# parthjaggi/flow

Hardware: AMD Instinct MI355X
Metric: env-steps/sec (higher is better)
Workload: dtype mixed

## Files before the change

flow_amd/csrc/flowsim_pair.h:

```cpp
#pragma once
#include "flowsim_kernels.h"

namespace fs {

typedef float f2 __attribute__((ext_vector_type(2)));
typedef unsigned u2v __attribute__((__vector_size__(8)));

enum : int { DPP_ROW_NEWBCAST0 = 0x150, DPP_ROW_NEWBCAST8 = 0x158 };

__device__ __forceinline__ f2 fma2(f2 a, f2 b, f2 c) { return __builtin_elementwise_fma(a, b, c); }
__device__ __forceinline__ f2 splat(float a) { return f2{a, a}; }

__device__ __forceinline__ f2 pk_mul(f2 a, f2 b) { return a * b; }
__device__ __forceinline__ f2 pk_add(f2 a, f2 b) { return a + b; }
__device__ __forceinline__ f2 pk_sub(f2 a, f2 b) { return a - b; }
__device__ __forceinline__ f2 pk_fma(f2 a, f2 b, f2 c) { return fma2(a, b, c); }
__device__ __forceinline__ f2 pk_fnma(f2 a, f2 b, f2 c) { return fma2(-a, b, c); }
__device__ __forceinline__ float nonneg_else(float x, float y) {
  const unsigned a = __builtin_bit_cast(unsigned, x), b = __builtin_bit_cast(unsigned, y);
  return __builtin_bit_cast(float, min(a, b));
}

template <int ROW>
__device__ __forceinline__ float next_a(float v, bool last, int lane) {
// ... 112 lines not shown
#define FS_PAIR_A_NZ_PARAM
#include "flowsim_pair_step_a_sm.inc"
#undef FS_PAIR_A_NAME
#undef FS_PAIR_A_NZ
#undef FS_PAIR_A_NZ_PARAM
#define FS_PAIR_A_NAME pair_step_asm_a_sm_nz
#define FS_PAIR_A_NZ 1
#define FS_PAIR_A_NZ_PARAM , f2 nz
#include "flowsim_pair_step_a_sm.inc"
#undef FS_PAIR_A_NAME
#undef FS_PAIR_A_NZ
#undef FS_PAIR_A_NZ_PARAM
__device__ __forceinline__ void pair_step_asm_b(f2& V, f2& X, f2& H, f2& DVL, f2& OV, unsigned& crash_bits, float& sq,
                                                const PairConsts& c) {
  asm volatile(
      "v_sub_f32_e32 v118, v112, v113\n"
      "v_sub_f32_e32 v132, v115, v114\n"
      "v_subrev_f32_dpp v119, v112, v113 row_shl:1 row_mask:0xf bank_mask:0xf bound_ctrl:1\n"
      "v_subrev_f32_dpp v134, v112, v113 row_newbcast:0 row_mask:0xf bank_mask:0xf\n"
      "v_sub_f32_dpp v133, v114, v115 row_shl:1 row_mask:0xf bank_mask:0xf bound_ctrl:1\n"
      "v_sub_f32_dpp v135, v114, v115 row_newbcast:0 row_mask:0xf bank_mask:0xf\n"
      "v_cndmask_b32_e64 v119, v119, v134, %[last]\n"
      "v_cndmask_b32_e64 v133, v133, v135, %[last]\n"
      "v_pk_add_f32 v[126:127], v[132:133], %[L2]\n"
      "v_min_u32_e32 v132, v132, v126\n"
      "v_min_u32_e32 v133, v133, v127\n"
      "v_pk_add_f32 v[116:117], v[132:133], %[lenlead] neg_lo:[0,1] neg_hi:[0,1]\n"
      "v_pk_add_f32 v[126:127], v[116:117], %[gap2] neg_lo:[0,1] neg_hi:[0,1]\n"
      "v_min_f32_e32 v126, v126, v127\n"
      "v_alignbit_b32 %[cb], %[cb], v126, 31\n"
      "v_pk_fma_f32 v[124:125], v[112:113], %[vmask], %[tvm]\n"
      "v_pk_mul_f32 v[124:125], v[124:125], v[124:125]\n"
      "v_add_f32_e32 %[sq], v124, v125\n"
      "v_cvt_f64_f32_e32 v[130:131], v112\n"
      "v_cvt_f64_f32_e32 v[132:133], v113\n"
      "v_mul_f64 v[134:135], v[130:131], %[rcms]\n"
      "v_mul_f64 v[136:137], v[132:133], %[rcms]\n"
      "v_fma_f64 v[130:131], -v[134:135], %[ms], v[130:131]\n"
      "v_fma_f64 v[132:133], -v[136:137], %[ms], v[132:133]\n"
      "v_fma_f64 v[134:135], v[130:131], %[rcms], v[134:135]\n"
      "v_fma_f64 v[136:137], v[132:133], %[rcms], v[136:137]\n"
      "v_cvt_f32_f64_e32 v128, v[134:135]\n"
      "v_cvt_f32_f64_e32 v129, v[136:137]\n"
      : "+{v[112:113]}"(V), "+{v[114:115]}"(X), "+{v[116:117]}"(H), "+{v[118:119]}"(DVL), "={v[128:129]}"(OV),
        [cb] "+v"(crash_bits), [sq] "=&v"(sq)
      : [L2] "v"(c.L2), [lenlead] "v"(c.len_lead), [gap2] "v"(c.gap2), [vmask] "v"(c.vmask), [tvm] "v"(c.tvm),
        [ms] "v"(c.ms64), [rcms] "v"(c.rc_ms64), [last] "s"(c.last_mask)
      : "v124", "v125", "v126", "v127", "v130", "v131", "v132", "v133", "v134", "v135", "v136", "v137");
}

struct MixedConsts {
  f2 p0, p1, p2, p5, rc_v0, tsab, rc_ab, one, gap2, vmask, tvm;
  float c1e3;
  double dt, ramp, L, rc_L, rc_ms, len_b, len_next, zero;
  unsigned long long last_mask;
};
__device__ __forceinline__ void mixed_step_asm_a(f2& V32, double& XA, double& XB, double& VA, double& VB, f2& H, f2& DVL,
                                                 f2& OV, const MixedConsts& c) {
  unsigned long long sa, sb;
  asm volatile(
      "v_cmp_nlt_f32_e64 %[sa], |v140|, %[c1e3]\n"
      "v_cmp_nlt_f32_e64 %[sb], |v141|, %[c1e3]\n"
      "v_pk_mul_f32 v[124:125], v[112:113], v[142:143]\n"
      "v_pk_mul_f32 v[126:127], v[124:125], %[rcab]\n"
      "v_pk_fma_f32 v[130:131], v[126:127], %[tsab], v[124:125] neg_lo:[1,0,0] neg_hi:[1,0,0]\n"
      "v_pk_fma_f32 v[126:127], v[130:131], %[rcab], v[126:127]\n"
      "v_cndmask_b32_e64 v120, %[c1e3], v140, %[sa]\n"
      "v_cndmask_b32_e64 v121, %[c1e3], v141, %[sb]\n"
      "v_pk_mul_f32 v[124:125], v[112:113], %[rcv0]\n"
      "v_rcp_f32_e32 v122, v120\n"
      "v_rcp_f32_e32 v123, v121\n"
      "v_pk_fma_f32 v[130:131], v[124:125], %[p0], v[112:113] neg_lo:[1,0,0] neg_hi:[1,0,0]\n"
      "v_pk_fma_f32 v[124:125], v[130:131], %[rcv0], v[124:125]\n"
      "v_pk_mul_f32 v[130:131], v[112:113], %[p1]\n"
      "v_pk_add_f32 v[130:131], v[130:131], v[126:127]\n"
      "v_pk_fma_f32 v[126:127], v[120:121], v[122:123], %[one] neg_lo:[1,0,0] neg_hi:[1,0,0]\n"
      "v_max_f32_e32 v130, 0, v130\n"
      "v_max_f32_e32 v131, 0, v131\n"
      "v_pk_fma_f32 v[122:123], v[126:127], v[122:123], v[122:123]\n"
      "v_pk_add_f32 v[130:131], %[p5], v[130:131]\n"
      "v_pk_mul_f32 v[124:125], v[124:125], v[124:125]\n"
      "v_pk_mul_f32 v[126:127], v[130:131], v[122:123]\n"
      "v_pk_mul_f32 v[124:125], v[124:125], v[124:125]\n"
      "v_pk_fma_f32 v[132:133], v[120:121], v[126:127], v[130:131] neg_lo:[1,0,0] neg_hi:[1,0,0]\n"
      "v_pk_add_f32 v[124:125], %[one], v[124:125] neg_lo:[0,1] neg_hi:[0,1]\n"
      "v_pk_fma_f32 v[126:127], v[132:133], v[122:123], v[126:127]\n"
      "v_pk_fma_f32 v[132:133], v[120:121], v[126:127], v[130:131] neg_lo:[1,0,0] neg_hi:[1,0,0]\n"
      "v_pk_fma_f32 v[126:127], v[132:133], v[122:123], v[126:127]\n"
      "v_pk_mul_f32 v[126:127], v[126:127], v[126:127]\n"
      "v_pk_add_f32 v[124:125], v[124:125], v[126:127] neg_lo:[0,1] neg_hi:[0,1]\n"
      "v_pk_mul_f32 v[124:125], %[p2], v[124:125]\n"
      "v_cvt_f64_f32_e32 v[130:131], v124\n"
      "v_cvt_f64_f32_e32 v[132:133], v125\n"
      "v_mul_f64 v[130:131], v[130:131], %[dt]\n"
      "v_mul_f64 v[132:133], v[132:133], %[dt]\n"
      "v_add_f64 v[130:131], v[118:119], v[130:131]\n"
      "v_add_f64 v[132:133], v[138:139], v[132:133]\n"
      "v_max_f64 v[130:131], v[130:131], %[zero]\n"
      "v_max_f64 v[132:133], v[132:133], %[zero]\n"
      "v_add_f64 v[130:131], v[130:131], -v[118:119]\n"
      "v_add_f64 v[132:133], v[132:133], -v[138:139]\n"
      "v_mul_f64 v[130:131], v[130:131], %[ramp]\n"
      "v_mul_f64 v[132:133], v[132:133], %[ramp]\n"
      "v_add_f64 v[118:119], v[118:119], v[130:131]\n"
      "v_add_f64 v[138:139], v[138:139], v[132:133]\n"
      "v_mul_f64 v[130:131], v[118:119], %[dt]\n"
      "v_mul_f64 v[132:133], v[138:139], %[dt]\n"
      "v_add_f64 v[130:131], v[114:115], v[130:131]\n"
      "v_add_f64 v[132:133], v[116:117], v[132:133]\n"
      "v_add_f64 v[134:135], v[130:131], -%[L]\n"
      "v_add_f64 v[136:137], v[132:133], -%[L]\n"
      "v_cvt_f32_f64_e32 v112, v[118:119]\n"
      "v_cvt_f32_f64_e32 v113, v[138:139]\n"
      "v_cmp_gt_i32_e64 %[sa], 0, v135\n"
      "v_cmp_gt_i32_e64 %[sb], 0, v137\n"
      "v_mul_f64 v[120:121], v[118:119], %[rcms]\n"
      "v_mul_f64 v[122:123], v[138:139], %[rcms]\n"
      "v_cndmask_b32_e64 v114, v134, v130, %[sa]\n"
      "v_cndmask_b32_e64 v115, v135, v131, %[sa]\n"
      "v_cndmask_b32_e64 v116, v136, v132, %[sb]\n"
      "v_cndmask_b32_e64 v117, v137, v133, %[sb]\n"
      "v_cvt_f32_f64_e32 v128, v[120:121]\n"
      "v_cvt_f32_f64_e32 v129, v[122:123]\n"
      : "+{v[112:113]}"(V32), "+{v[114:115]}"(XA), "+{v[116:117]}"(XB), "+{v[118:119]}"(VA), "+{v[138:139]}"(VB),
        "+{v[140:141]}"(H), "+{v[142:143]}"(DVL), "={v[128:129]}"(OV), [sa] "=&s"(sa), [sb] "=&s"(sb)
      : [c1e3] "v"(c.c1e3), [rcab] "v"(c.rc_ab), [tsab] "v"(c.tsab), [rcv0] "v"(c.rc_v0), [p0] "v"(c.p0),
        [p1] "v"(c.p1), [p2] "v"(c.p2), [p5] "v"(c.p5), [one] "v"(c.one), [dt] "v"(c.dt), [ramp] "v"(c.ramp),
        [L] "v"(c.L), [rcms] "v"(c.rc_ms), [zero] "v"(c.zero)
      : "v120", "v121", "v122", "v123", "v124", "v125", "v126", "v127", "v130", "v131", "v132", "v133", "v134",
        "v135", "v136", "v137");
}
struct MixedSumoConsts { double fl0a, fl0b, adta, adtb, ddta, ddtb; };
__device__ __forceinline__ void mixed_step_asm_a_sm(f2& V32, double& XA, double& XB, double& VA, double& VB, f2& H,
                                                    f2& DVL, f2& OV, const MixedConsts& c, const SumoPair& m,
                                                    const MixedSumoConsts& d) {
  unsigned long long sa, sb;
  asm volatile(
      "v_cmp_nlt_f32_e64 %[sa], |v140|, %[c1e3]\n"
      "v_cmp_nlt_f32_e64 %[sb], |v141|, %[c1e3]\n"
      "v_pk_mul_f32 v[124:125], v[112:113], v[142:143]\n"
      "v_pk_mul_f32 v[126:127], v[124:125], %[rcab]\n"
      "v_pk_mul_f32 v[150:151], v[124:125], %[rcts]\n"
      "v_pk_fma_f32 v[130:131], v[126:127], %[tsab], v[124:125] neg_lo:[1,0,0] neg_hi:[1,0,0]\n"
      "v_pk_fma_f32 v[152:153], v[150:151], %[ts], v[124:125] neg_lo:[1,0,0] neg_hi:[1,0,0]\n"
      "v_pk_fma_f32 v[126:127], v[130:131], %[rcab], v[126:127]\n"
      "v_pk_fma_f32 v[150:151], v[152:153], %[rcts], v[150:151]\n"
      "v_cndmask_b32_e64 v120, %[c1e3], v140, %[sa]\n"
      "v_cndmask_b32_e64 v121, %[c1e3], v141, %[sb]\n"
      "v_max_f32_e32 v146, v140, %[c1e3]\n"
      "v_max_f32_e32 v147, v141, %[c1e3]\n"
      "v_pk_mul_f32 v[124:125], v[112:113], %[rcv0]\n"
      "v_rcp_f32_e32 v122, v120\n"
      "v_rcp_f32_e32 v123, v121\n"
      "v_rcp_f32_e32 v148, v146\n"
      "v_rcp_f32_e32 v149, v147\n"
      "v_pk_fma_f32 v[130:131], v[124:125], %[p0], v[112:113] neg_lo:[1,0,0] neg_hi:[1,0,0]\n"
      "v_pk_mul_f32 v[154:155], v[112:113], %[rcsm]\n"
      "v_pk_fma_f32 v[124:125], v[130:131], %[rcv0], v[124:125]\n"
      "v_pk_fma_f32 v[152:153], v[154:155], %[smax], v[112:113] neg_lo:[1,0,0] neg_hi:[1,0,0]\n"
      "v_pk_mul_f32 v[130:131], v[112:113], %[p1]\n"
      "v_pk_fma_f32 v[154:155], v[152:153], %[rcsm], v[154:155]\n"
      "v_pk_add_f32 v[130:131], v[130:131], v[126:127]\n"
      "v_pk_mul_f32 v[152:153], v[112:113], %[tau]\n"
      "v_pk_fma_f32 v[126:127], v[120:121], v[122:123], %[one] neg_lo:[1,0,0] neg_hi:[1,0,0]\n"
      "v_pk_add_f32 v[150:151], v[152:153], v[150:151]\n"
      "v_pk_fma_f32 v[152:153], v[146:147], v[148:149], %[one] neg_lo:[1,0,0] neg_hi:[1,0,0]\n"
      "v_max_f32_e32 v130, 0, v130\n"
      "v_max_f32_e32 v131, 0, v131\n"
      "v_max_f32_e32 v150, 0, v150\n"
      "v_max_f32_e32 v151, 0, v151\n"
      "v_pk_fma_f32 v[122:123], v[126:127], v[122:123], v[122:123]\n"
      "v_pk_fma_f32 v[148:149], v[152:153], v[148:149], v[148:149]\n"
      "v_pk_add_f32 v[130:131], %[p5], v[130:131]\n"
      "v_pk_add_f32 v[150:151], %[mgap], v[150:151]\n"
      "v_pk_mul_f32 v[124:125], v[124:125], v[124:125]\n"
      "v_pk_mul_f32 v[154:155], v[154:155], v[154:155]\n"
      "v_pk_mul_f32 v[126:127], v[130:131], v[122:123]\n"
      "v_pk_mul_f32 v[152:153], v[150:151], v[148:149]\n"
      "v_pk_mul_f32 v[124:125], v[124:125], v[124:125]\n"
      "v_pk_mul_f32 v[154:155], v[154:155], v[154:155]\n"
      "v_pk_fma_f32 v[132:133], v[120:121], v[126:127], v[130:131] neg_lo:[1,0,0] neg_hi:[1,0,0]\n"
      "v_pk_fma_f32 v[134:135], v[146:147], v[152:153], v[150:151] neg_lo:[1,0,0] neg_hi:[1,0,0]\n"
      "v_pk_add_f32 v[124:125], %[one], v[124:125] neg_lo:[0,1] neg_hi:[0,1]\n"
      "v_pk_add_f32 v[154:155], %[one], v[154:155] neg_lo:[0,1] neg_hi:[0,1]\n"
      "v_pk_fma_f32 v[126:127], v[132:133], v[122:123], v[126:127]\n"
      "v_pk_fma_f32 v[152:153], v[134:135], v[148:149], v[152:153]\n"
      "v_pk_fma_f32 v[132:133], v[120:121], v[126:127], v[130:131] neg_lo:[1,0,0] neg_hi:[1,0,0]\n"
      "v_pk_fma_f32 v[134:135], v[146:147], v[152:153], v[150:151] neg_lo:[1,0,0] neg_hi:[1,0,0]\n"
      "v_pk_fma_f32 v[126:127], v[132:133], v[122:123], v[126:127]\n"
      "v_pk_fma_f32 v[152:153], v[134:135], v[148:149], v[152:153]\n"
      "v_pk_mul_f32 v[126:127], v[126:127], v[126:127]\n"
      "v_pk_mul_f32 v[152:153], v[152:153], v[152:153]\n"
      "v_pk_add_f32 v[124:125], v[124:125], v[126:127] neg_lo:[0,1] neg_hi:[0,1]\n"
      "v_pk_add_f32 v[154:155], v[154:155], v[152:153] neg_lo:[0,1] neg_hi:[0,1]\n"
      "v_pk_mul_f32 v[124:125], %[p2], v[124:125]\n"
      "v_pk_mul_f32 v[154:155], %[maxa], v[154:155]\n"
      "v_cvt_f64_f32_e32 v[130:131], v124\n"
      "v_cvt_f64_f32_e32 v[132:133], v125\n"
      "v_cvt_f64_f32_e32 v[134:135], v154\n"
      "v_cvt_f64_f32_e32 v[136:137], v155\n"
      "v_mul_f64 v[130:131], v[130:131], %[dt]\n"
      "v_mul_f64 v[132:133], v[132:133], %[dt]\n"
      "v_mul_f64 v[134:135], v[134:135], %[dt]\n"
      "v_mul_f64 v[136:137], v[136:137], %[dt]\n"
      "v_add_f64 v[130:131], v[118:119], v[130:131]\n"
      "v_add_f64 v[132:133], v[138:139], v[132:133]\n"
      "v_add_f64 v[134:135], v[118:119], v[134:135]\n"
      "v_add_f64 v[136:137], v[138:139], v[136:137]\n"
      "v_max_f64 v[130:131], v[130:131], %[zero]\n"
      "v_max_f64 v[132:133], v[132:133], %[zero]\n"
      "v_max_f64 v[134:135], v[134:135], %[fl0a]\n"
      "v_max_f64 v[136:137], v[136:137], %[fl0b]\n"
      "v_add_f64 v[130:131], v[130:131], -v[118:119]\n"
      "v_add_f64 v[132:133], v[132:133], -v[138:139]\n"
      "v_mul_f64 v[130:131], v[130:131], %[ramp]\n"
      "v_mul_f64 v[132:133], v[132:133], %[ramp]\n"
      "v_add_f64 v[130:131], v[118:119], v[130:131]\n"
      "v_add_f64 v[132:133], v[138:139], v[132:133]\n"
      "v_min_f64 v[130:131], v[130:131], v[134:135]\n"
      "v_min_f64 v[132:133], v[132:133], v[136:137]\n"
      "v_add_f64 v[134:135], v[118:119], %[adta]\n"
      "v_add_f64 v[136:137], v[138:139], %[adtb]\n"
      "v_min_f64 v[130:131], v[130:131], v[134:135]\n"
      "v_min_f64 v[132:133], v[132:133], v[136:137]\n"
      "v_add_f64 v[134:135], v[118:119], -%[ddta]\n"
      "v_add_f64 v[136:137], v[138:139], -%[ddtb]\n"
      "v_max_f64 v[118:119], v[130:131], v[134:135]\n"
      "v_max_f64 v[138:139], v[132:133], v[136:137]\n"
      "v_mul_f64 v[130:131], v[118:119], %[dt]\n"
      "v_mul_f64 v[132:133], v[138:139], %[dt]\n"
      "v_add_f64 v[130:131], v[114:115], v[130:131]\n"
      "v_add_f64 v[132:133], v[116:117], v[132:133]\n"
      "v_add_f64 v[134:135], v[130:131], -%[L]\n"
      "v_add_f64 v[136:137], v[132:133], -%[L]\n"
      "v_cvt_f32_f64_e32 v112, v[118:119]\n"
      "v_cvt_f32_f64_e32 v113, v[138:139]\n"
      "v_cmp_gt_i32_e64 %[sa], 0, v135\n"
      "v_cmp_gt_i32_e64 %[sb], 0, v137\n"
      "v_mul_f64 v[120:121], v[118:119], %[rcms]\n"
      "v_mul_f64 v[122:123], v[138:139], %[rcms]\n"
      "v_cndmask_b32_e64 v114, v134, v130, %[sa]\n"
      "v_cndmask_b32_e64 v115, v135, v131, %[sa]\n"
      "v_cndmask_b32_e64 v116, v136, v132, %[sb]\n"
      "v_cndmask_b32_e64 v117, v137, v133, %[sb]\n"
      "v_cvt_f32_f64_e32 v128, v[120:121]\n"
      "v_cvt_f32_f64_e32 v129, v[122:123]\n"
      : "+{v[112:113]}"(V32), "+{v[114:115]}"(XA), "+{v[116:117]}"(XB), "+{v[118:119]}"(VA), "+{v[138:139]}"(VB),
        "+{v[140:141]}"(H), "+{v[142:143]}"(DVL), "={v[128:129]}"(OV), [sa] "=&s"(sa), [sb] "=&s"(sb)
      : [c1e3] "v"(c.c1e3), [rcab] "v"(c.rc_ab), [tsab] "v"(c.tsab), [rcv0] "v"(c.rc_v0), [p0] "v"(c.p0),
        [p1] "v"(c.p1), [p2] "v"(c.p2), [p5] "v"(c.p5), [one] "v"(c.one), [dt] "v"(c.dt), [ramp] "v"(c.ramp),
        [L] "v"(c.L), [rcms] "v"(c.rc_ms), [zero] "v"(c.zero), [rcts] "v"(m.rc_ts), [ts] "v"(m.ts),
        [rcsm] "v"(m.rc_smax), [smax] "v"(m.smax), [tau] "v"(m.tau), [mgap] "v"(m.min_gap), [maxa] "v"(m.maxa),
        [fl0a] "v"(d.fl0a), [fl0b] "v"(d.fl0b), [adta] "v"(d.adta), [adtb] "v"(d.adtb), [ddta] "v"(d.ddta),
        [ddtb] "v"(d.ddtb)
      : "v120", "v121", "v122", "v123", "v124", "v125", "v126", "v127", "v130", "v131", "v132", "v133", "v134",
        "v135", "v136", "v137", "v146", "v147", "v148", "v149", "v150", "v151", "v152", "v153", "v154", "v155");
}
__device__ __forceinline__ void mixed_step_asm_b(f2& V32, double& XA, double& XB, f2& H, f2& DVL, f2& OX,
                                                 unsigned& crash_bits, float& sq, const MixedConsts& c) {
  unsigned long long sa, sb;
  asm volatile(
      "v_sub_f32_e32 v142, v112, v113\n"
      "v_subrev_f32_dpp v143, v112, v113 row_shl:1 row_mask:0xf bank_mask:0xf bound_ctrl:1\n"
      "v_subrev_f32_dpp v124, v112, v113 row_newbcast:0 row_mask:0xf bank_mask:0xf\n"
      "v_mov_b32_dpp v130, v114 row_shl:1 row_mask:0xf bank_mask:0xf bound_ctrl:1\n"
      "v_mov_b32_dpp v131, v115 row_shl:1 row_mask:0xf bank_mask:0xf bound_ctrl:1\n"
      "v_mov_b32_dpp v132, v114 row_newbcast:0 row_mask:0xf bank_mask:0xf\n"
      "v_mov_b32_dpp v133, v115 row_newbcast:0 row_mask:0xf bank_mask:0xf\n"
      "v_cndmask_b32_e64 v143, v143, v124, %[last]\n"
      "v_cndmask_b32_e64 v130, v130, v132, %[last]\n"
      "v_cndmask_b32_e64 v131, v131, v133, %[last]\n"
      "v_mul_f64 v[120:121], v[114:115], %[rcL]\n"
      "v_mul_f64 v[122:123], v[116:117], %[rcL]\n"
      "v_add_f64 v[134:135], v[116:117], -v[114:115]\n"
      "v_add_f64 v[136:137], v[130:131], -v[116:117]\n"
      "v_cvt_f32_f64_e32 v144, v[120:121]\n"
      "v_cvt_f32_f64_e32 v145, v[122:123]\n"
      "v_add_f64 v[130:131], v[134:135], %[L]\n"
      "v_add_f64 v[132:133], v[136:137], %[L]\n"
      "v_cmp_gt_i32_e64 %[sa], 0, v135\n"
      "v_cmp_gt_i32_e64 %[sb], 0, v137\n"
      "v_pk_fma_f32 v[124:125], v[112:113], %[vmask], %[tvm]\n"
      "v_pk_mul_f32 v[124:125], v[124:125], v[124:125]\n"
      "v_cndmask_b32_e64 v134, v134, v130, %[sa]\n"
      "v_cndmask_b32_e64 v135, v135, v131, %[sa]\n"
      "v_cndmask_b32_e64 v136, v136, v132, %[sb]\n"
      "v_cndmask_b32_e64 v137, v137, v133, %[sb]\n"
      "v_add_f32_e32 %[sq], v124, v125\n"
      "v_add_f64 v[134:135], v[134:135], -%[lenb]\n"
      "v_add_f64 v[136:137], v[136:137], -%[lennext]\n"
      "v_cvt_f32_f64_e32 v140, v[134:135]\n"
      "v_cvt_f32_f64_e32 v141, v[136:137]\n"
      "v_pk_add_f32 v[126:127], v[140:141], %[gap2] neg_lo:[0,1] neg_hi:[0,1]\n"
      "v_min_f32_e32 v126, v126, v127\n"
      "v_alignbit_b32 %[cb], %[cb], v126, 31\n"
      : "+{v[112:113]}"(V32), "+{v[114:115]}"(XA), "+{v[116:117]}"(XB), "+{v[140:141]}"(H), "+{v[142:143]}"(DVL),
        "={v[144:145]}"(OX), [cb] "+v"(crash_bits), [sq] "=&v"(sq), [sa] "=&s"(sa), [sb] "=&s"(sb)
      : [L] "v"(c.L), [rcL] "v"(c.rc_L), [gap2] "v"(c.gap2), [vmask] "v"(c.vmask), [tvm] "v"(c.tvm),
        [lenb] "v"(c.len_b), [lennext] "v"(c.len_next), [last] "s"(c.last_mask)
      : "v120", "v121", "v122", "v123", "v124", "v125", "v126", "v127", "v130", "v131", "v132", "v133", "v134",
        "v135", "v136", "v137");
}

template <typename T, int ROW, bool DELTA4, bool FASTDIV, bool BADCHK, bool SM = false, bool NOISE = false>
__global__ __launch_bounds__(256) void k_rollout_pair(DevView<T> s, int num_steps, float* __restrict__ obs,
                                                      float* __restrict__ rew, uint8_t* __restrict__ done) {
  constexpr bool MIXED = sizeof(T) == 8;
  static_assert(!(NOISE && MIXED), "FS_MIXED has no noise form (its C twin cannot reproduce the hardware's log / cos)");
  constexpr bool ASM = ROW == 16 && DELTA4 && FASTDIV && !BADCHK;
  constexpr int RPW = 64 / ROW;
  constexpr int PERIOD = ROW < 16 ? ROW : 16;
  const int lane = threadIdx.x & 63;
  const int wave = (blockIdx.x * blockDim.x + threadIdx.x) >> 6;
  const int row = lane / ROW;
  const int k = lane % ROW;
  const int r = wave * RPW + row;
  const int N = s.N;
  const int LP = N >> 1;
  const bool rvalid = r < s.R;
  const bool valid = rvalid && k < LP;
  const int rr = rvalid ? r : s.R - 1;
  const int kk = k < LP ? k : LP - 1;
  const bool last = (kk == LP - 1);
  const int iA = 2 * kk, iB = iA + 1;
  const size_t idx = size_t(rr) * N + iA;

  f2 p[6];
#pragma unroll
  for (int q = 0; q < 6; ++q) p[q] = f2{float(s.p[q * N + iA]), float(s.p[q * N + iB])};
  const T lenB = s.length[iB];
  const T len_nextA = next_a<ROW>(T(s.length[iA]), last, lane);
  const T base_len = s.ring_len[rr];
  const T L = base_len + T(4) * s.jlen;
  int tcount = s.time[rr];
  uint32_t nctr = NOISE ? s.noise_ctr[rr] : 0u;
  const f2 sigma = NOISE ? f2{float(s.noise[iA]), float(s.noise[iB])} : f2{0.0f, 0.0f};
  const bool noisyA = NOISE && sigma.x > 0.0f, noisyB = NOISE && sigma.y > 0.0f;
  float gA[4] = {0.0f, 0.0f, 0.0f, 0.0f}, gB[4] = {0.0f, 0.0f, 0.0f, 0.0f};
  if constexpr (NOISE) {
    if ((nctr & 3u) != 0u) {
      gauss4<float>(s.seed_lo, s.seed_hi, s.rep0 + uint32_t(rr), uint32_t(iA), nctr >> 2, gA, s.noise_exact != 0);
      gauss4<float>(s.seed_lo, s.seed_hi, s.rep0 + uint32_t(rr), uint32_t(iB), nctr >> 2, gB, s.noise_exact != 0);
      for (uint32_t q = 0; q < (nctr & 3u); ++q) {
        gA[0] = gA[1]; gA[1] = gA[2]; gA[2] = gA[3];
        gB[0] = gB[1]; gB[1] = gB[2]; gB[2] = gB[3];
      }
    }
  }

  const float dt = float(s.dt), ramp = float(s.ramp);
  const f2 two_sqrt_ab = {2.0f * tsqrt(p[2].x * p[3].x), 2.0f * tsqrt(p[2].y * p[3].y)};
  const f2 rc_v0 = {1.0f / p[0].x, 1.0f / p[0].y}, rc_ab = {1.0f / two_sqrt_ab.x, 1.0f / two_sqrt_ab.y};
  const float Lf = float(L);
  const f2 L2 = splat(Lf), rc_L2 = splat(1.0f / Lf), one = splat(1.0f), dt2 = splat(dt), ramp2 = splat(ramp);
  const f2 gap2 = splat(float(s.crash_gap)), m100 = splat(-100.0f);
  const f2 vmask = splat(valid ? 1.0f : 0.0f), tvm = splat(valid ? -float(s.target_velocity) : 0.0f);
  const double ms64 = double(s.max_speed), rc_ms64 = 1.0 / ms64;
  const double L64 = double(L), rc_L64 = 1.0 / L64, dt64 = double(s.dt), ramp64 = double(s.ramp);

  f2 x, v;
  double xdA = 0, xdB = 0, vdA = 0, vdB = 0;
  if (MIXED) {
    xdA = double(s.pos[idx]); xdB = double(s.pos[idx + 1]);
    vdA = double(s.vel[idx]); vdB = double(s.vel[idx + 1]);
    v = f2{float(vdA), float(vdB)};
    x = f2{0.0f, 0.0f};
  } else {
    x = f2{float(s.pos[idx]), float(s.pos[idx + 1])};
    v = f2{float(s.vel[idx]), float(s.vel[idx + 1])};
  }
  const f2 len_lead = {float(lenB), float(len_nextA)};

  auto headway = [&]() -> f2 {
    if (MIXED) {
      const double xn = next_a<ROW>(xdA, last, lane);
      double dA = xdB - xdA, dB = xn - xdB;
      dA = dA < 0.0 ? dA + L64 : dA;
      dB = dB < 0.0 ? dB + L64 : dB;
      return f2{float(dA - double(lenB)), float(dB - double(len_nextA))};
    } else {
      const f2 xl = {x.y, next_a<ROW>(x.x, last, lane)};
      f2 d = pk_sub(xl, x);
      const f2 dw = pk_add(d, L2);
      d.x = nonneg_else(d.x, dw.x);
      d.y = nonneg_else(d.y, dw.y);
      return pk_sub(d, len_lead);
    }
  };
  f2 h = headway();
  f2 vl = {v.y, next_a<ROW>(v.x, last, lane)};
  f2 dvl = v - vl;
  PairConsts pc;
  pc.p0 = p[0]; pc.p1 = p[1]; pc.p2 = p[2]; pc.p5 = p[5]; pc.rc_v0 = rc_v0; pc.tsab = two_sqrt_ab; pc.rc_ab = rc_ab;
  pc.one = one; pc.dt2 = dt2; pc.ramp2 = ramp2; pc.L2 = L2; pc.rc_L2 = rc_L2; pc.len_lead = len_lead;
  pc.gap2 = gap2; pc.vmask = vmask; pc.tvm = tvm; pc.c1e3 = 1e-3f; pc.ms64 = ms64; pc.rc_ms64 = rc_ms64;
  pc.last_mask = __ballot(last);
  MixedConsts mc;
  mc.p0 = p[0]; mc.p1 = p[1]; mc.p2 = p[2]; mc.p5 = p[5]; mc.rc_v0 = rc_v0; mc.tsab = two_sqrt_ab; mc.rc_ab = rc_ab;
  mc.one = one; mc.gap2 = gap2; mc.vmask = vmask; mc.tvm = tvm; mc.c1e3 = 1e-3f; mc.dt = dt64; mc.ramp = ramp64;
  mc.L = L64; mc.rc_L = rc_L64; mc.rc_ms = rc_ms64; mc.len_b = double(lenB); mc.len_next = double(len_nextA);
  mc.zero = 0.0; mc.last_mask = pc.last_mask;
  SumoPair sc{};
  double floor0A = 0, floor0B = 0, adtA = 0, adtB = 0, ddtA = 0, ddtB = 0;
  if constexpr (SM) {
    const int mA = s.speed_mode[iA], mB = s.speed_mode[iB];
    const float maA = float(s.max_accel[iA]), maB = float(s.max_accel[iB]);
    const float mdA = float(s.max_decel[iA]), mdB = float(s.max_decel[iB]);
    sc.tau = f2{float(s.sumo_tau[iA]), float(s.sumo_tau[iB])};
    sc.min_gap = f2{float(s.sumo_min_gap[iA]), float(s.sumo_min_gap[iB])};
    sc.maxa = f2{maA, maB};
    sc.smax = f2{float(s.sumo_max_speed[iA]), float(s.sumo_max_speed[iB])};
    sc.rc_smax = f2{1.0f / sc.smax.x, 1.0f / sc.smax.y};
    sc.ts = f2{2.0f * tsqrt(maA * mdA), 2.0f * tsqrt(maB * mdB)};
    sc.rc_ts = f2{1.0f / sc.ts.x, 1.0f / sc.ts.y};
    const float BIG = 3.0e38f;
    sc.floor0 = f2{(mA & 1) ? 0.0f : BIG, (mB & 1) ? 0.0f : BIG};
    sc.adt = f2{(mA & 2) ? maA * dt : BIG, (mB & 2) ? maB * dt : BIG};
    sc.ddt = f2{(mA & 4) ? mdA * dt : BIG, (mB & 4) ? mdB * dt : BIG};
    floor0A = double(sc.floor0.x); floor0B = double(sc.floor0.y);
    adtA = (mA & 2) ? double(s.max_accel[iA]) * dt64 : double(BIG);
    adtB = (mB & 2) ? double(s.max_accel[iB]) * dt64 : double(BIG);
    ddtA = (mA & 4) ? double(s.max_decel[iA]) * dt64 : double(BIG);
    ddtB = (mB & 4) ? double(s.max_decel[iB]) * dt64 : double(BIG);
  }
  const MixedSumoConsts msc = {floor0A, floor0B, adtA, adtB, ddtA, ddtB};

  const unsigned rowb = 2u * unsigned(N) * 4u;
  const unsigned off_v = unsigned(rr) * rowb + unsigned(iA) * 4u;
  const unsigned off_x = off_v + unsigned(N) * 4u;
  const size_t step_bytes = size_t(s.R) * rowb;
  const unsigned step_b32 = unsigned(step_bytes);
  char* ob = reinterpret_cast<char*>(obs);
  unsigned crash_bits = 0u, bad_bits = 0u;

  typedef unsigned u4v __attribute__((__vector_size__(16)));
  constexpr bool XPOSE = ASM;
  __shared__ float row_img[XPOSE ? 4 : 1][XPOSE ? RPW * 64 : 1];
  float* const my_img = row_img[XPOSE ? (threadIdx.x >> 6) & 3 : 0] + (XPOSE ? row * 2 * N : 0);
  const unsigned off_16 = unsigned(rr) * rowb + unsigned(kk) * 16u;
  u4v piece = {0u, 0u, 0u, 0u};
  auto transpose_in = [&](f2 ov, f2 ox) {
    *reinterpret_cast<f2*>(my_img + 2 * kk) = ov;
    *reinterpret_cast<f2*>(my_img + N + 2 * kk) = ox;
    __builtin_amdgcn_fence(__ATOMIC_RELEASE, "wavefront");
    __builtin_amdgcn_wave_barrier();
    __builtin_amdgcn_fence(__ATOMIC_ACQUIRE, "wavefront");
    piece = *reinterpret_cast<const u4v*>(my_img + 4 * kk);
  };

  auto noise_term = [&]() -> f2 {
    f2 nz = {-0.0f, -0.0f};
    if constexpr (NOISE) {
      const bool fresh = (nctr & 3u) == 0u;
      if (__ballot(fresh) != 0ull) {
        if (fresh) {
          gauss4<float>(s.seed_lo, s.seed_hi, s.rep0 + uint32_t(rr), uint32_t(iA), nctr >> 2, gA, s.noise_exact != 0);
          gauss4<float>(s.seed_lo, s.seed_hi, s.rep0 + uint32_t(rr), uint32_t(iB), nctr >> 2, gB, s.noise_exact != 0);
        }
      }
      const float tA = sigma.x * gA[0], tB = sigma.y * gB[0];
      nz.x = noisyA ? tA : -0.0f;
      nz.y = noisyB ? tB : -0.0f;
      gA[0] = gA[1]; gA[1] = gA[2]; gA[2] = gA[3];
      gB[0] = gB[1]; gB[1] = gB[2]; gB[2] = gB[3];
      nctr += 1u;
    }
    return nz;
  };

  auto one_step = [&](int slot, __amdgpu_buffer_rsrc_t rs, float& sq_out) {
    if constexpr (ASM) {
      f2 ov, ox;
      const unsigned so = unsigned(slot) * step_b32;
      if constexpr (MIXED) {
        if constexpr (SM) mixed_step_asm_a_sm(v, xdA, xdB, vdA, vdB, h, dvl, ov, mc, sc, msc);
        else mixed_step_asm_a(v, xdA, xdB, vdA, vdB, h, dvl, ov, mc);
        if (slot > 0) __builtin_amdgcn_raw_buffer_store_b128(piece, rs, off_16, so - step_b32, 0);
        mixed_step_asm_b(v, xdA, xdB, h, dvl, ox, crash_bits, sq_out, mc);
        transpose_in(ov, ox);
      } else {
#if defined(FS_DIAG_NOSTORE)
        pair_step_asm_a(v, x, h, dvl, ox, pc);
        pair_step_asm_b(v, x, h, dvl, ov, crash_bits, sq_out, pc);
        asm volatile("" :: "v"(ov), "v"(ox), "s"(so));
#elif defined(FS_DIAG_NOXPOSE)
        pair_step_asm_a(v, x, h, dvl, ox, pc);
        __builtin_amdgcn_raw_buffer_store_b64(__builtin_bit_cast(u2v, ox), rs, off_x, so, 0);
        pair_step_asm_b(v, x, h, dvl, ov, crash_bits, sq_out, pc);
        __builtin_amdgcn_raw_buffer_store_b64(__builtin_bit_cast(u2v, ov), rs, off_v, so, 0);
#else
        if constexpr (NOISE) {
          const f2 nz = noise_term();
          if constexpr (SM) pair_step_asm_a_sm_nz(v, x, h, dvl, ox, pc, sc, nz);
          else pair_step_asm_a_nz(v, x, h, dvl, ox, pc, nz);
        } else {
          if constexpr (SM) pair_step_asm_a_sm(v, x, h, dvl, ox, pc, sc);
          else pair_step_asm_a(v, x, h, dvl, ox, pc);
        }
        if (slot > 0) __builtin_amdgcn_raw_buffer_store_b128(piece, rs, off_16, so - step_b32, 0);
        pair_step_asm_b(v, x, h, dvl, ov, crash_bits, sq_out, pc);
        transpose_in(ov, ox);
#endif
      }
      return;
    }
    f2 acc = idm_pair<DELTA4, FASTDIV>(v, vl, h, p, two_sqrt_ab, rc_ab, rc_v0, one);
    if constexpr (NOISE) acc = pk_add(acc, noise_term());
    f2 acc_s = {0.0f, 0.0f};
    if constexpr (SM) acc_s = sumo_acc_pair<FASTDIV>(v, vl, h, sc, one);
    f2 ox;
    if (MIXED) {
      const double aA = double(acc.x), aB = double(acc.y);
      const double nA = tmax(vdA + aA * dt64, 0.0), nB = tmax(vdB + aB * dt64, 0.0);
      double cA = vdA + (nA - vdA) * ramp64, cB = vdB + (nB - vdB) * ramp64;
      if constexpr (SM) {
        const double sA = tmax(vdA + double(acc_s.x) * dt64, floor0A), sB = tmax(vdB + double(acc_s.y) * dt64, floor0B);
        cA = tmin(cA, sA); cB = tmin(cB, sB);
        cA = tmin(cA, vdA + adtA); cB = tmin(cB, vdB + adtB);
        cA = tmax(cA, vdA - ddtA); cB = tmax(cB, vdB - ddtB);
      }
      vdA = cA;
      vdB = cB;
      const double xA = xdA + vdA * dt64, xB = xdB + vdB * dt64;
      xdA = xA >= L64 ? xA - L64 : xA;
      xdB = xB >= L64 ? xB - L64 : xB;
      v = f2{float(vdA), float(vdB)};
      ox = f2{float(xdA * rc_L64), float(xdB * rc_L64)};
    } else {
      f2 nv = pk_add(v, pk_mul(acc, dt2));
      nv.x = tmax(nv.x, 0.0f);
      nv.y = tmax(nv.y, 0.0f);
      f2 vc = pk_add(v, pk_mul(pk_sub(nv, v), ramp2));
      if constexpr (SM) {
        const f2 vs = pk_add(v, pk_mul(acc_s, dt2));
        const f2 cap1 = pk_add(v, sc.adt), flo = pk_sub(v, sc.ddt);
        vc.x = tmin(vc.x, tmax(sc.floor0.x, vs.x));
        vc.y = tmin(vc.y, tmax(sc.floor0.y, vs.y));
        vc.x = tmax(tmin(vc.x, cap1.x), flo.x);
        vc.y = tmax(tmin(vc.y, cap1.y), flo.y);
      }
      v = vc;
      const f2 xn = pk_add(x, pk_mul(v, dt2));
      const f2 xw = pk_sub(xn, L2);
      x.x = nonneg_else(xw.x, xn.x);
      x.y = nonneg_else(xw.y, xn.y);
      ox = div_const2<FASTDIV>(x, L2, rc_L2);
    }
    h = headway();
    vl = f2{v.y, next_a<ROW>(v.x, last, lane)};
    const f2 hc = pk_sub(h, gap2);
    crash_bits = __builtin_amdgcn_alignbit(crash_bits, __builtin_bit_cast(unsigned, __builtin_fminf(hc.x, hc.y)), 31);
    if (BADCHK) {
      const f2 vb = pk_sub(v, m100);
      bad_bits = __builtin_amdgcn_alignbit(bad_bits, __builtin_bit_cast(unsigned, __builtin_fminf(vb.x, vb.y)), 31);
    }
    f2 ov;
    if (MIXED) ov = f2{float(vdA * rc_ms64), float(vdB * rc_ms64)};
    else ov = f2{div_via_f64(v.x, ms64, rc_ms64), div_via_f64(v.y, ms64, rc_ms64)};
    const unsigned so = unsigned(slot) * step_b32;
    __builtin_amdgcn_raw_buffer_store_b64(__builtin_bit_cast(u2v, ov), rs, off_v, so, 0);
    __builtin_amdgcn_raw_buffer_store_b64(__builtin_bit_cast(u2v, ox), rs, off_x, so, 0);
    const f2 dv = pk_fma(v, vmask, tvm);
    const f2 sq = pk_mul(dv, dv);
    sq_out = sq.x + sq.y;
  };

  int base = 0;
  for (; base + PERIOD <= num_steps; base += PERIOD) {
    float sq[PERIOD];
    const size_t remain = size_t(num_steps - base) * step_bytes;
    const __amdgpu_buffer_rsrc_t rs = __builtin_amdgcn_make_buffer_rsrc(
        ob, 0, remain > 0xFFFFFFFFull ? 0xFFFFFFFFu : unsigned(remain), 0x00020000);
#pragma unroll
    for (int slot = 0; slot < PERIOD; ++slot) one_step(slot, rs, sq[slot]);
#if !defined(FS_DIAG_NOSTORE) && !defined(FS_DIAG_NOXPOSE)
    if (XPOSE) __builtin_amdgcn_raw_buffer_store_b128(piece, rs, off_16, unsigned(PERIOD - 1) * step_b32, 0);
#endif
    ob += size_t(PERIOD) * step_bytes;
    tcount += PERIOD;
    const float racc = transposed_sum<ROW, PERIOD>(sq, lane);
    const unsigned crash_any = seg_or<ROW>(crash_bits);
    const unsigned bad_any = (BADCHK ? seg_or<ROW>(bad_bits) : 0u) | crash_any;
    crash_bits = 0u;
    bad_bits = 0u;
    if (rvalid && k < PERIOD) {
      const bool my_crash = (crash_any >> (PERIOD - 1 - k)) & 1u;
      const bool my_bad = (bad_any >> (PERIOD - 1 - k)) & 1u;
      const int t_k = tcount - (PERIOD - 1 - k);
      const float cost = tsqrt(racc);
      const float max_cost = float(s.max_cost);
      float reward = tmax(max_cost - cost, 0.0f) / (max_cost + 1.1920928955078125e-07f);
      reward = my_bad ? 0.0f : reward;
      const size_t o = size_t(base + k) * s.R + rr;
      rew[o] = reward;
      done[o] = done_flag(t_k >= s.step_limit, my_crash);
    }
  }
#pragma unroll 1
  for (; base < num_steps; ++base) {
    float sq1;
    const __amdgpu_buffer_rsrc_t rs = __builtin_amdgcn_make_buffer_rsrc(ob, 0, unsigned(step_bytes), 0x00020000);
    one_step(0, rs, sq1);
#if !defined(FS_DIAG_NOSTORE) && !defined(FS_DIAG_NOXPOSE)
    if (XPOSE) __builtin_amdgcn_raw_buffer_store_b128(piece, rs, off_16, 0u, 0);
#endif
    ob += step_bytes;
    tcount += 1;
    const float racc = seg_sum<ROW>(sq1);
    const bool my_crash = (seg_or<ROW>(crash_bits) & 1u) != 0u;
    const bool my_bad = (BADCHK && (seg_or<ROW>(bad_bits) & 1u) != 0u) || my_crash;
    crash_bits = 0u;
    bad_bits = 0u;
    if (rvalid && k == 0) {
      const float cost = tsqrt(racc);
      const float max_cost = float(s.max_cost);
      float reward = tmax(max_cost - cost, 0.0f) / (max_cost + 1.1920928955078125e-07f);
      reward = my_bad ? 0.0f : reward;
      const size_t o = size_t(base) * s.R + rr;
      rew[o] = reward;
      done[o] = done_flag(tcount >= s.step_limit, my_crash);
    }
  }
  if (valid) {
    if (MIXED) {
      s.pos[idx] = T(xdA); s.pos[idx + 1] = T(xdB);
      s.vel[idx] = T(vdA); s.vel[idx + 1] = T(vdB);
    } else {
      s.pos[idx] = T(x.x); s.pos[idx + 1] = T(x.y);
      s.vel[idx] = T(v.x); s.vel[idx + 1] = T(v.y);
    }
    if (kk == 0) s.time[rr] = tcount;
    if (NOISE && kk == 0) s.noise_ctr[rr] = nctr;
  }
}

template <typename T>
__global__ void k_obs_mixed(DevView<T> s, float* __restrict__ obs) {
  if constexpr (std::is_same<T, double>::value) {
    const int e = blockIdx.x * blockDim.x + threadIdx.x;
    if (e >= s.R * s.N) return;
    const int r = e / s.N, i = e % s.N;
    const double L = s.ring_len[r] + 4.0 * s.jlen;
    float* o = obs + size_t(r) * 2 * s.N;
    o[i] = float(s.vel[e] * (1.0 / double(s.max_speed)));
    o[s.N + i] = float(s.pos[e] * (1.0 / L));
  }
}

}
```

Baseline: 13.77 billion.

## Batch LDS transposes over step pairs and streamline mixed-precision wrap logic

The mixed-precision pair kernel now stages two consecutive steps into a doubled LDS image and transposes them with one wave barrier per pair. The buffer stores for the even and odd steps are deferred by two slots, with an explicit waitcnt. The position wrap replaces the subtract-plus-integer-compare-plus-cndmask sequence with an f64 compare feeding an fma against a synthesized 0/1 multiplier. The gap wrap uses a med3 trick on the high word to build a scale factor, and the neighbour shift uses DPP cndmask. Together these aim to cut LDS barrier and instruction counts, at the cost of more LDS, more registers, and subtle bit-level wrap arithmetic that must stay exact.

```diff
diff --git a/flow_amd/csrc/flowsim_pair.h b/flow_amd/csrc/flowsim_pair.h
--- a/flow_amd/csrc/flowsim_pair.h
+++ b/flow_amd/csrc/flowsim_pair.h
@@ -188,12 +188,14 @@
 struct MixedConsts {
   f2 p0, p1, p2, p5, rc_v0, tsab, rc_ab, one, gap2, vmask, tvm;
   float c1e3;
-  double dt, ramp, L, rc_L, rc_ms, len_b, len_next, zero;
+  unsigned one_hi, wrap_hi;
+  double dt, ramp, L, rc_L, rc_ms, len_b, len_next, zero, L_wrap;
   unsigned long long last_mask;
 };
 __device__ __forceinline__ void mixed_step_asm_a(f2& V32, double& XA, double& XB, double& VA, double& VB, f2& H, f2& DVL,
-                                                 f2& OV, const MixedConsts& c) {
+                                                 f2& OV, double& WA, double& WB, const MixedConsts& c) {
   unsigned long long sa, sb;
+  float ova, ovb;
   asm volatile(
       "v_cmp_nlt_f32_e64 %[sa], |v140|, %[c1e3]\n"
       "v_cmp_nlt_f32_e64 %[sb], |v141|, %[c1e3]\n"
@@ -244,33 +246,33 @@
       "v_mul_f64 v[132:133], v[138:139], %[dt]\n"
       "v_add_f64 v[130:131], v[114:115], v[130:131]\n"
       "v_add_f64 v[132:133], v[116:117], v[132:133]\n"
-      "v_add_f64 v[134:135], v[130:131], -%[L]\n"
-      "v_add_f64 v[136:137], v[132:133], -%[L]\n"
+      "v_cmp_ge_f64_e64 %[sa], v[130:131], %[L]\n"
+      "v_cmp_ge_f64_e64 %[sb], v[132:133], %[L]\n"
       "v_cvt_f32_f64_e32 v112, v[118:119]\n"
       "v_cvt_f32_f64_e32 v113, v[138:139]\n"
-      "v_cmp_gt_i32_e64 %[sa], 0, v135\n"
-      "v_cmp_gt_i32_e64 %[sb], 0, v137\n"
+      "v_cndmask_b32_e64 v157, 0, %[onehi], %[sa]\n"
+      "v_cndmask_b32_e64 v159, 0, %[onehi], %[sb]\n"
       "v_mul_f64 v[120:121], v[118:119], %[rcms]\n"
       "v_mul_f64 v[122:123], v[138:139], %[rcms]\n"
-      "v_cndmask_b32_e64 v114, v134, v130, %[sa]\n"
-      "v_cndmask_b32_e64 v115, v135, v131, %[sa]\n"
-      "v_cndmask_b32_e64 v116, v136, v132, %[sb]\n"
-      "v_cndmask_b32_e64 v117, v137, v133, %[sb]\n"
-      "v_cvt_f32_f64_e32 v128, v[120:121]\n"
-      "v_cvt_f32_f64_e32 v129, v[122:123]\n"
+      "v_fma_f64 v[114:115], -%[L], v[156:157], v[130:131]\n"
+      "v_fma_f64 v[116:117], -%[L], v[158:159], v[132:133]\n"
+      "v_cvt_f32_f64_e32 %[ova], v[120:121]\n"
+      "v_cvt_f32_f64_e32 %[ovb], v[122:123]\n"
       : "+{v[112:113]}"(V32), "+{v[114:115]}"(XA), "+{v[116:117]}"(XB), "+{v[118:119]}"(VA), "+{v[138:139]}"(VB),
-        "+{v[140:141]}"(H), "+{v[142:143]}"(DVL), "={v[128:129]}"(OV), [sa] "=&s"(sa), [sb] "=&s"(sb)
+        "+{v[140:141]}"(H), "+{v[142:143]}"(DVL), [ova] "=&v"(ova), [ovb] "=&v"(ovb), "+{v[156:157]}"(WA),
+        "+{v[158:159]}"(WB), [sa] "=&s"(sa), [sb] "=&s"(sb)
       : [c1e3] "v"(c.c1e3), [rcab] "v"(c.rc_ab), [tsab] "v"(c.tsab), [rcv0] "v"(c.rc_v0), [p0] "v"(c.p0),
         [p1] "v"(c.p1), [p2] "v"(c.p2), [p5] "v"(c.p5), [one] "v"(c.one), [dt] "v"(c.dt), [ramp] "v"(c.ramp),
-        [L] "v"(c.L), [rcms] "v"(c.rc_ms), [zero] "v"(c.zero)
-      : "v120", "v121", "v122", "v123", "v124", "v125", "v126", "v127", "v130", "v131", "v132", "v133", "v134",
-        "v135", "v136", "v137");
+        [L] "v"(c.L), [rcms] "v"(c.rc_ms), [zero] "v"(c.zero), [onehi] "v"(c.one_hi)
+      : "v120", "v121", "v122", "v123", "v124", "v125", "v126", "v127", "v130", "v131", "v132", "v133");
+  OV = f2{ova, ovb};
 }
 struct MixedSumoConsts { double fl0a, fl0b, adta, adtb, ddta, ddtb; };
 __device__ __forceinline__ void mixed_step_asm_a_sm(f2& V32, double& XA, double& XB, double& VA, double& VB, f2& H,
-                                                    f2& DVL, f2& OV, const MixedConsts& c, const SumoPair& m,
-                                                    const MixedSumoConsts& d) {
+                                                    f2& DVL, f2& OV, double& WA, double& WB, const MixedConsts& c,
+                                                    const SumoPair& m, const MixedSumoConsts& d) {
   unsigned long long sa, sb;
+  float ova, ovb;
   asm volatile(
       "v_cmp_nlt_f32_e64 %[sa], |v140|, %[c1e3]\n"
       "v_cmp_nlt_f32_e64 %[sb], |v141|, %[c1e3]\n"
@@ -367,61 +369,55 @@
       "v_mul_f64 v[132:133], v[138:139], %[dt]\n"
       "v_add_f64 v[130:131], v[114:115], v[130:131]\n"
       "v_add_f64 v[132:133], v[116:117], v[132:133]\n"
-      "v_add_f64 v[134:135], v[130:131], -%[L]\n"
-      "v_add_f64 v[136:137], v[132:133], -%[L]\n"
+      "v_cmp_ge_f64_e64 %[sa], v[130:131], %[L]\n"
+      "v_cmp_ge_f64_e64 %[sb], v[132:133], %[L]\n"
       "v_cvt_f32_f64_e32 v112, v[118:119]\n"
       "v_cvt_f32_f64_e32 v113, v[138:139]\n"
-      "v_cmp_gt_i32_e64 %[sa], 0, v135\n"
-      "v_cmp_gt_i32_e64 %[sb], 0, v137\n"
+      "v_cndmask_b32_e64 v157, 0, %[onehi], %[sa]\n"
+      "v_cndmask_b32_e64 v159, 0, %[onehi], %[sb]\n"
       "v_mul_f64 v[120:121], v[118:119], %[rcms]\n"
       "v_mul_f64 v[122:123], v[138:139], %[rcms]\n"
-      "v_cndmask_b32_e64 v114, v134, v130, %[sa]\n"
-      "v_cndmask_b32_e64 v115, v135, v131, %[sa]\n"
-      "v_cndmask_b32_e64 v116, v136, v132, %[sb]\n"
-      "v_cndmask_b32_e64 v117, v137, v133, %[sb]\n"
-      "v_cvt_f32_f64_e32 v128, v[120:121]\n"
-      "v_cvt_f32_f64_e32 v129, v[122:123]\n"
+      "v_fma_f64 v[114:115], -%[L], v[156:157], v[130:131]\n"
+      "v_fma_f64 v[116:117], -%[L], v[158:159], v[132:133]\n"
+      "v_cvt_f32_f64_e32 %[ova], v[120:121]\n"
+      "v_cvt_f32_f64_e32 %[ovb], v[122:123]\n"
       : "+{v[112:113]}"(V32), "+{v[114:115]}"(XA), "+{v[116:117]}"(XB), "+{v[118:119]}"(VA), "+{v[138:139]}"(VB),
-        "+{v[140:141]}"(H), "+{v[142:143]}"(DVL), "={v[128:129]}"(OV), [sa] "=&s"(sa), [sb] "=&s"(sb)
+        "+{v[140:141]}"(H), "+{v[142:143]}"(DVL), [ova] "=&v"(ova), [ovb] "=&v"(ovb), "+{v[156:157]}"(WA),
+        "+{v[158:159]}"(WB), [sa] "=&s"(sa), [sb] "=&s"(sb)
       : [c1e3] "v"(c.c1e3), [rcab] "v"(c.rc_ab), [tsab] "v"(c.tsab), [rcv0] "v"(c.rc_v0), [p0] "v"(c.p0),
         [p1] "v"(c.p1), [p2] "v"(c.p2), [p5] "v"(c.p5), [one] "v"(c.one), [dt] "v"(c.dt), [ramp] "v"(c.ramp),
-        [L] "v"(c.L), [rcms] "v"(c.rc_ms), [zero] "v"(c.zero), [rcts] "v"(m.rc_ts), [ts] "v"(m.ts),
+        [L] "v"(c.L), [rcms] "v"(c.rc_ms), [zero] "v"(c.zero), [onehi] "v"(c.one_hi), [rcts] "v"(m.rc_ts), [ts] "v"(m.ts),
         [rcsm] "v"(m.rc_smax), [smax] "v"(m.smax), [tau] "v"(m.tau), [mgap] "v"(m.min_gap), [maxa] "v"(m.maxa),
         [fl0a] "v"(d.fl0a), [fl0b] "v"(d.fl0b), [adta] "v"(d.adta), [adtb] "v"(d.adtb), [ddta] "v"(d.ddta),
         [ddtb] "v"(d.ddtb)
       : "v120", "v121", "v122", "v123", "v124", "v125", "v126", "v127", "v130", "v131", "v132", "v133", "v134",
         "v135", "v136", "v137", "v146", "v147", "v148", "v149", "v150", "v151", "v152", "v153", "v154", "v155");
-}
-__device__ __forceinline__ void mixed_step_asm_b(f2& V32, double& XA, double& XB, f2& H, f2& DVL, f2& OX,
-                                                 unsigned& crash_bits, float& sq, const MixedConsts& c) {
-  unsigned long long sa, sb;
+  OV = f2{ova, ovb};
+}
+__device__ __forceinline__ void mixed_step_asm_b(f2& V32, double& XA, double& XB, f2& H, f2& DVL, f2& OX, double& WA,
+                                                 double& WB, unsigned& crash_bits, float& sq, const MixedConsts& c) {
+  float oxa, oxb;
   asm volatile(
+      "s_mov_b64 vcc, %[last]\n"
       "v_sub_f32_e32 v142, v112, v113\n"
-      "v_subrev_f32_dpp v143, v112, v113 row_shl:1 row_mask:0xf bank_mask:0xf bound_ctrl:1\n"
-      "v_subrev_f32_dpp v124, v112, v113 row_newbcast:0 row_mask:0xf bank_mask:0xf\n"
-      "v_mov_b32_dpp v130, v114 row_shl:1 row_mask:0xf bank_mask:0xf bound_ctrl:1\n"
-      "v_mov_b32_dpp v131, v115 row_shl:1 row_mask:0xf bank_mask:0xf bound_ctrl:1\n"
-      "v_mov_b32_dpp v132, v114 row_newbcast:0 row_mask:0xf bank_mask:0xf\n"
-      "v_mov_b32_dpp v133, v115 row_newbcast:0 row_mask:0xf bank_mask:0xf\n"
-      "v_cndmask_b32_e64 v143, v143, v124, %[last]\n"
-      "v_cndmask_b32_e64 v130, v130, v132, %[last]\n"
-      "v_cndmask_b32_e64 v131, v131, v133, %[last]\n"
+      "v_mov_b32_dpp v124, v112 row_newbcast:0 row_mask:0xf bank_mask:0xf\n"
+      "v_mov_b64_dpp v[132:133], v[114:115] row_newbcast:0 row_mask:0xf bank_mask:0xf\n"
+      "v_cndmask_b32_dpp v124, v112, v124, vcc row_shl:1 row_mask:0xf bank_mask:0xf bound_ctrl:1\n"
+      "v_cndmask_b32_dpp v130, v114, v132, vcc row_shl:1 row_mask:0xf bank_mask:0xf bound_ctrl:1\n"
+      "v_cndmask_b32_dpp v131, v115, v133, vcc row_shl:1 row_mask:0xf bank_mask:0xf bound_ctrl:1\n"
       "v_mul_f64 v[120:121], v[114:115], %[rcL]\n"
       "v_mul_f64 v[122:123], v[116:117], %[rcL]\n"
       "v_add_f64 v[134:135], v[116:117], -v[114:115]\n"
       "v_add_f64 v[136:137], v[130:131], -v[116:117]\n"
-      "v_cvt_f32_f64_e32 v144, v[120:121]\n"
-      "v_cvt_f32_f64_e32 v145, v[122:123]\n"
-      "v_add_f64 v[130:131], v[134:135], %[L]\n"
-      "v_add_f64 v[132:133], v[136:137], %[L]\n"
-      "v_cmp_gt_i32_e64 %[sa], 0, v135\n"
-      "v_cmp_gt_i32_e64 %[sb], 0, v137\n"
+      "v_sub_f32_e32 v143, v113, v124\n"
+      "v_cvt_f32_f64_e32 %[oxa], v[120:121]\n"
+      "v_cvt_f32_f64_e32 %[oxb], v[122:123]\n"
+      "v_med3_i32 v157, v135, %[wraphi], 0\n"
+      "v_med3_i32 v159, v137, %[wraphi], 0\n"
       "v_pk_fma_f32 v[124:125], v[112:113], %[vmask], %[tvm]\n"
       "v_pk_mul_f32 v[124:125], v[124:125], v[124:125]\n"
-      "v_cndmask_b32_e64 v134, v134, v130, %[sa]\n"
-      "v_cndmask_b32_e64 v135, v135, v131, %[sa]\n"
-      "v_cndmask_b32_e64 v136, v136, v132, %[sb]\n"
-      "v_cndmask_b32_e64 v137, v137, v133, %[sb]\n"
+      "v_fma_f64 v[134:135], %[Lwrap], v[156:157], v[134:135]\n"
+      "v_fma_f64 v[136:137], %[Lwrap], v[158:159], v[136:137]\n"
       "v_add_f32_e32 %[sq], v124, v125\n"
       "v_add_f64 v[134:135], v[134:135], -%[lenb]\n"
       "v_add_f64 v[136:137], v[136:137], -%[lennext]\n"
@@ -431,11 +427,13 @@
       "v_min_f32_e32 v126, v126, v127\n"
       "v_alignbit_b32 %[cb], %[cb], v126, 31\n"
       : "+{v[112:113]}"(V32), "+{v[114:115]}"(XA), "+{v[116:117]}"(XB), "+{v[140:141]}"(H), "+{v[142:143]}"(DVL),
-        "={v[144:145]}"(OX), [cb] "+v"(crash_bits), [sq] "=&v"(sq), [sa] "=&s"(sa), [sb] "=&s"(sb)
-      : [L] "v"(c.L), [rcL] "v"(c.rc_L), [gap2] "v"(c.gap2), [vmask] "v"(c.vmask), [tvm] "v"(c.tvm),
-        [lenb] "v"(c.len_b), [lennext] "v"(c.len_next), [last] "s"(c.last_mask)
-      : "v120", "v121", "v122", "v123", "v124", "v125", "v126", "v127", "v130", "v131", "v132", "v133", "v134",
+        [oxa] "=&v"(oxa), [oxb] "=&v"(oxb), "+{v[156:157]}"(WA), "+{v[158:159]}"(WB), [cb] "+v"(crash_bits),
+        [sq] "=&v"(sq)
+      : [rcL] "v"(c.rc_L), [gap2] "v"(c.gap2), [vmask] "v"(c.vmask), [tvm] "v"(c.tvm), [lenb] "v"(c.len_b),
+        [lennext] "v"(c.len_next), [wraphi] "v"(c.wrap_hi), [Lwrap] "v"(c.L_wrap), [last] "s"(c.last_mask)
+      : "vcc", "v120", "v121", "v122", "v123", "v124", "v125", "v126", "v127", "v130", "v131", "v132", "v133", "v134",
         "v135", "v136", "v137");
+  OX = f2{oxa, oxb};
 }
 
 template <typename T, int ROW, bool DELTA4, bool FASTDIV, bool BADCHK, bool SM = false, bool NOISE = false>
@@ -536,6 +534,10 @@
   mc.one = one; mc.gap2 = gap2; mc.vmask = vmask; mc.tvm = tvm; mc.c1e3 = 1e-3f; mc.dt = dt64; mc.ramp = ramp64;
   mc.L = L64; mc.rc_L = rc_L64; mc.rc_ms = rc_ms64; mc.len_b = double(lenB); mc.len_next = double(len_nextA);
   mc.zero = 0.0; mc.last_mask = pc.last_mask;
+  const unsigned wrap_exp = (unsigned(__builtin_bit_cast(unsigned long long, L64) >> 32) & 0x7FF00000u) + 0x02000000u;
+  mc.one_hi = 0x3FF00000u; mc.wrap_hi = 0x80000000u | wrap_exp;
+  mc.L_wrap = -L64 * __builtin_bit_cast(double, (unsigned long long)(0x7FE00000u - wrap_exp) << 32);
+  double wA = 0.0, wB = 0.0;
   SumoPair sc{};
   double floor0A = 0, floor0B = 0, adtA = 0, adtB = 0, ddtA = 0, ddtB = 0;
   if constexpr (SM) {
@@ -571,8 +573,15 @@
 
   typedef unsigned u4v __attribute__((__vector_size__(16)));
   constexpr bool XPOSE = ASM;
-  __shared__ float row_img[XPOSE ? 4 : 1][XPOSE ? RPW * 64 : 1];
-  float* const my_img = row_img[XPOSE ? (threadIdx.x >> 6) & 3 : 0] + (XPOSE ? row * 2 * N : 0);
+#if defined(FS_DIAG_NOSTAGE2)
+  constexpr bool XPOSE2 = false;
+#else
+  constexpr bool XPOSE2 = XPOSE && MIXED;
+#endif
+  __shared__ float row_img[XPOSE ? 4 : 1][XPOSE ? RPW * 64 * (XPOSE2 ? 2 : 1) : 1];
+  float* const my_wave_img = row_img[XPOSE ? (threadIdx.x >> 6) & 3 : 0];
+  float* const my_img = my_wave_img + (XPOSE ? row * 2 * N : 0);
+  float* const my_img2 = my_wave_img + (XPOSE2 ? row * 4 * N : 0);
   const unsigned off_16 = unsigned(rr) * rowb + unsigned(kk) * 16u;
   u4v piece = {0u, 0u, 0u, 0u};
   auto transpose_in = [&](f2 ov, f2 ox) {
@@ -582,6 +591,23 @@
     __builtin_amdgcn_wave_barrier();
     __builtin_amdgcn_fence(__ATOMIC_ACQUIRE, "wavefront");
     piece = *reinterpret_cast<const u4v*>(my_img + 4 * kk);
+  };
+  typedef float f4 __attribute__((ext_vector_type(4)));
+  f2 ov_even = {0.0f, 0.0f}, ox_even = {0.0f, 0.0f};
+  u4v piece_even = {0u, 0u, 0u, 0u}, piece_odd = {0u, 0u, 0u, 0u};
+  int odd_at = 8 * kk + 2;
+  asm volatile("" : "+v"(odd_at));
+  auto transpose_in2 = [&](f2 ov, f2 ox) {
+    *reinterpret_cast<f4*>(my_img2 + 4 * kk) = f4{ov_even.x, ov_even.y, ov.x, ov.y};
+    *reinterpret_cast<f4*>(my_img2 + 2 * N + 4 * kk) = f4{ox_even.x, ox_even.y, ox.x, ox.y};
+    __builtin_amdgcn_fence(__ATOMIC_RELEASE, "wavefront");
+    __builtin_amdgcn_wave_barrier();
+    __builtin_amdgcn_fence(__ATOMIC_ACQUIRE, "wavefront");
+    const u2v* const qe = reinterpret_cast<const u2v*>(my_img2 + 8 * kk);
+    const u2v* const qo = reinterpret_cast<const u2v*>(my_img2 + odd_at);
+    const u2v e0 = qe[0], e1 = qe[2], o0 = qo[0], o1 = qo[2];
+    piece_even = u4v{e0[0], e0[1], e1[0], e1[1]};
+    piece_odd = u4v{o0[0], o0[1], o1[0], o1[1]};
   };
 
   auto noise_term = [&]() -> f2 {
@@ -604,16 +630,28 @@
     return nz;
   };
 
-  auto one_step = [&](int slot, __amdgpu_buffer_rsrc_t rs, float& sq_out) {
+  auto one_step = [&](int slot, __amdgpu_buffer_rsrc_t rs, float& sq_out, bool in_block) {
     if constexpr (ASM) {
       f2 ov, ox;
       const unsigned so = unsigned(slot) * step_b32;
       if constexpr (MIXED) {
-        if constexpr (SM) mixed_step_asm_a_sm(v, xdA, xdB, vdA, vdB, h, dvl, ov, mc, sc, msc);
-        else mixed_step_asm_a(v, xdA, xdB, vdA, vdB, h, dvl, ov, mc);
-        if (slot > 0) __builtin_amdgcn_raw_buffer_store_b128(piece, rs, off_16, so - step_b32, 0);
-        mixed_step_asm_b(v, xdA, xdB, h, dvl, ox, crash_bits, sq_out, mc);
-        transpose_in(ov, ox);
+        if constexpr (SM) mixed_step_asm_a_sm(v, xdA, xdB, vdA, vdB, h, dvl, ov, wA, wB, mc, sc, msc);
+        else mixed_step_asm_a(v, xdA, xdB, vdA, vdB, h, dvl, ov, wA, wB, mc);
+        if (in_block && XPOSE2) {
+          if (slot > 1 && !(slot & 1)) __builtin_amdgcn_s_waitcnt(0xC07F);
+          if (slot > 1) __builtin_amdgcn_raw_buffer_store_b128((slot & 1) ? piece_odd : piece_even, rs, off_16, so - 2u * step_b32, 0);
+        } else if (slot > 0) {
+          __builtin_amdgcn_raw_buffer_store_b128(piece, rs, off_16, so - step_b32, 0);
+        }
+        mixed_step_asm_b(v, xdA, xdB, h, dvl, ox, wA, wB, crash_bits, sq_out, mc);
+        if (!in_block || !XPOSE2) {
+          transpose_in(ov, ox);
+        } else if (slot & 1) {
+          transpose_in2(ov, ox);
+        } else {
+          ov_even = ov;
+          ox_even = ox;
+        }
       } else {
 #if defined(FS_DIAG_NOSTORE)
         pair_step_asm_a(v, x, h, dvl, ox, pc);
@@ -708,9 +746,14 @@
     const __amdgpu_buffer_rsrc_t rs = __builtin_amdgcn_make_buffer_rsrc(
         ob, 0, remain > 0xFFFFFFFFull ? 0xFFFFFFFFu : unsigned(remain), 0x00020000);
 #pragma unroll
-    for (int slot = 0; slot < PERIOD; ++slot) one_step(slot, rs, sq[slot]);
+    for (int slot = 0; slot < PERIOD; ++slot) one_step(slot, rs, sq[slot], true);
 #if !defined(FS_DIAG_NOSTORE) && !defined(FS_DIAG_NOXPOSE)
-    if (XPOSE) __builtin_amdgcn_raw_buffer_store_b128(piece, rs, off_16, unsigned(PERIOD - 1) * step_b32, 0);
+    if (XPOSE2) {
+      __builtin_amdgcn_raw_buffer_store_b128(piece_even, rs, off_16, unsigned(PERIOD - 2) * step_b32, 0);
+      __builtin_amdgcn_raw_buffer_store_b128(piece_odd, rs, off_16, unsigned(PERIOD - 1) * step_b32, 0);
+    } else if (XPOSE) {
+      __builtin_amdgcn_raw_buffer_store_b128(piece, rs, off_16, unsigned(PERIOD - 1) * step_b32, 0);
+    }
 #endif
     ob += size_t(PERIOD) * step_bytes;
     tcount += PERIOD;
@@ -736,7 +779,7 @@
   for (; base < num_steps; ++base) {
     float sq1;
     const __amdgpu_buffer_rsrc_t rs = __builtin_amdgcn_make_buffer_rsrc(ob, 0, unsigned(step_bytes), 0x00020000);
-    one_step(0, rs, sq1);
+    one_step(0, rs, sq1, false);
 #if !defined(FS_DIAG_NOSTORE) && !defined(FS_DIAG_NOXPOSE)
     if (XPOSE) __builtin_amdgcn_raw_buffer_store_b128(piece, rs, off_16, 0u, 0);
 #endif
```

After: 13.66 billion. No clear change (-0.8%).
